# itshawi/data-accelerator

Hardware: AMD Instinct MI355X
Metric: events/sec (node) + p99 latency, SimulatedData IoT Flow (higher is better)
Workload: dtype fp64/int64 columns (no reduced precision)

## Files before the change

### dxa/ops/csrc/inflate.hip

```cpp
#include "dxa_common.h"

namespace {

constexpr int IG = 16;
constexpr int WG = 128;
constexpr int LBITS = 9;
constexpr int DBITS = 8;
constexpr int kWaitVm0 = 0xF70;

enum : int32_t { IF_OK = 0, IF_TRUNC = 1, IF_DIST = 2, IF_OVERFLOW = 3, IF_SIZE = 4, IF_CODE = 10, IF_BLOCK = 6 };

struct Tables {
  uint16_t lfast[1 << LBITS];
  uint16_t dfast[1 << DBITS];
  uint16_t lsorted[288];
  uint16_t dsorted[32];
  uint16_t lcount[16];
  uint16_t dcount[16];
  uint8_t lens[320];
  uint8_t clens[20];
  uint16_t csorted[19];
  uint16_t ccount[16];
};

__constant__ uint16_t kLenBase[29] = {3,  4,  5,  6,  7,  8,  9,  10, 11,  13,  15,  17,  19,  23, 27,
                                      31, 35, 43, 51, 59, 67, 83, 99, 115, 131, 163, 195, 227, 258};
__constant__ uint8_t kLenExtra[29] = {0, 0, 0, 0, 0, 0, 0, 0, 1, 1, 1, 1, 2, 2, 2, 2, 3, 3, 3, 3, 4, 4, 4, 4, 5, 5, 5, 5, 0};
__constant__ uint16_t kDistBase[30] = {1,   2,   3,   4,   5,   7,    9,    13,   17,   25,   33,   49,    65,    97,    129,
                                       193, 257, 385, 513, 769, 1025, 1537, 2049, 3073, 4097, 6145, 8193, 12289, 16385, 24577};
__constant__ uint8_t kDistExtra[30] = {0, 0, 0, 0, 1, 1, 2, 2, 3, 3, 4, 4, 5, 5, 6, 6, 7, 7, 8, 8, 9, 9, 10, 10, 11, 11, 12, 12, 13, 13};
__constant__ uint8_t kClenOrder[19] = {16, 17, 18, 0, 8, 7, 9, 6, 10, 5, 11, 4, 12, 3, 13, 2, 14, 1, 15};

__device__ __forceinline__ uint32_t bitrev(uint32_t c, int n) { return __builtin_bitreverse32(c) >> (32 - n); }

__device__ __forceinline__ void lane_sync() {
  __builtin_amdgcn_fence(__ATOMIC_RELEASE, "wavefront");
  __builtin_amdgcn_wave_barrier();
  __builtin_amdgcn_fence(__ATOMIC_ACQUIRE, "wavefront");
}

__device__ bool build_table(const uint8_t* lens, int n, uint16_t* count, uint16_t* sorted, uint16_t* fast, int bits,
                            int maxlen, int gl) {
  lane_sync();
  if (fast) {
    for (int i = gl; i < (1 << bits); i += IG) fast[i] = 0;
    lane_sync();
  }
  uint16_t cnt[16];
  for (int l = 0; l < 16; ++l) cnt[l] = 0;
  for (int s = 0; s < n; ++s) cnt[lens[s]]++;
  int left = 1;
  for (int l = 1; l <= maxlen; ++l) {
    left = (left << 1) - cnt[l];
    if (left < 0) return false;
  }
  uint16_t offs[16];
  offs[1] = 0;
  for (int l = 1; l < 15; ++l) offs[l + 1] = offs[l] + cnt[l];
  if (gl == 0) {
    for (int l = 0; l < 16; ++l) count[l] = cnt[l];
  }
  uint32_t next[16];
  uint32_t code = 0;
  next[0] = 0;
  for (int l = 1; l < 16; ++l) {
    next[l] = code;
    code = (code + cnt[l]) << 1;
  }
  for (int s = 0; s < n; ++s) {
    const int l = lens[s];
    if (!l) continue;
    if (gl == 0) sorted[offs[l]] = (uint16_t)s;
    offs[l]++;
    const uint32_t c = next[l]++;
    if (fast && l <= bits) {
      const uint32_t r = bitrev(c, l);
      const uint16_t e = (uint16_t)((l << 9) | s);
      for (int k = gl; k < (1 << (bits - l)); k += IG) fast[r | ((uint32_t)k << l)] = e;
    }
  }
  lane_sync();
  return true;
}

__global__ __launch_bounds__(WG) void inflate_group_kernel(const uint8_t* __restrict__ src,
                                                           const int64_t* __restrict__ comp_off,
                                                           const int32_t* __restrict__ comp_len,
                                                           const uint8_t* __restrict__ kind,
                                                           const int64_t* __restrict__ out_off,
                                                           const int64_t* __restrict__ cap_arr, int64_t nb,
                                                           uint8_t* __restrict__ dst, int64_t* __restrict__ produced,
                                                           int32_t* __restrict__ status) {
  __shared__ Tables tabs[WG / IG];
  Tables& T = tabs[threadIdx.x / IG];
  const int64_t b = ((int64_t)blockIdx.x * WG + threadIdx.x) / IG;
  const int gl = (int)(threadIdx.x & (IG - 1));
  if (b >= nb || kind[b] != 2) return;
  const uint8_t* in = src + comp_off[b];
  const int32_t n = comp_len[b];
  const int64_t cap64 = cap_arr[b];
  uint8_t* out = dst + out_off[b];
  if (n < 0 || cap64 < 0 || cap64 > INT32_MAX) {
    if (gl == 0) status[b] = IF_OVERFLOW;
    return;
  }
  const int32_t cap = (int32_t)cap64;
  const int32_t lim = n + 8;
  uint64_t bb = 0;
  int bc = 0;
  int32_t ip = 0;
  auto ld32 = [&](int32_t p) -> uint32_t {
    if (p + 4 <= lim) {
      const uintptr_t a = reinterpret_cast<uintptr_t>(in + p);
      const uint32_t* w = reinterpret_cast<const uint32_t*>(a & ~(uintptr_t)3);
      const uint32_t sh = (uint32_t)(a & 3) * 8u;
      const uint32_t lo = w[0];
      if (!sh) return lo;
      return (lo >> sh) | (w[1] << (32u - sh));
    }
    uint32_t v = 0;
    for (int i = 0; i < 4; ++i)
      if (p + i < lim) v |= (uint32_t)in[p + i] << (8 * i);
    return v;
  };
  auto refill = [&]() {
    if (bc <= 32) {
      bb |= (uint64_t)ld32(ip) << bc;
      ip += 4;
      bc += 32;
    }
  };
  auto bits = [&](int k) -> uint32_t {
    refill();
    const uint32_t v = (uint32_t)(bb & ((1ull << k) - 1));
    bb >>= k;
    bc -= k;
    return v;
  };
  auto slow = [&](const uint16_t* count, const uint16_t* sorted, int maxlen) -> int {
    refill();
    int code = 0, first = 0, index = 0;
    for (int l = 1; l <= maxlen; ++l) {
      code |= (int)(bb & 1);
      bb >>= 1;
      bc--;
      const int c = count[l];
      if (code - first < c) return sorted[index + code - first];
      index += c;
      first = (first + c) << 1;
      code <<= 1;
    }
    return -1;
  };
  auto decode = [&](const uint16_t* fast, int fbits, const uint16_t* count, const uint16_t* sorted) -> int {
    refill();
    const uint32_t e = fast[bb & ((1u << fbits) - 1)];
    const int l = (int)(e >> 9);
    if (l) {
      bb >>= l;
      bc -= l;
      return (int)(e & 511);
    }
    return slow(count, sorted, 15);
  };
  int32_t op = 0, rc = IF_OK, done = 0;
  bool last = false;
  while (!last && rc == IF_OK) {
    if ((int64_t)ip * 8 - bc > (int64_t)lim * 8) { rc = IF_TRUNC; break; }
    last = bits(1) != 0;
    const uint32_t type = bits(2);
    if (type == 0) {
      const int drop = bc & 7;
      bb >>= drop;
      bc -= drop;
      const uint32_t len = bits(16), nlen = bits(16);
      if ((len ^ 0xffffu) != nlen) { rc = IF_BLOCK; break; }
      const int32_t pos = ip - bc / 8;
      if (pos + (int32_t)len > n) { rc = IF_TRUNC; break; }
      if (op + (int32_t)len > cap) { rc = IF_OVERFLOW; break; }
      for (int32_t c = gl; c < (int32_t)len; c += IG) out[op + c] = in[pos + c];
      op += (int32_t)len;
      ip = pos + (int32_t)len;
      bb = 0;
      bc = 0;
      continue;
    }
    if (type == 3) { rc = IF_BLOCK; break; }
    int nlit = 288, ndist = 30;
    if (type == 1) {
      for (int s = gl; s < 320; s += IG) T.lens[s] = s < 144 ? 8 : s < 256 ? 9 : s < 280 ? 7 : s < 288 ? 8 : 5;
    } else {
      nlit = (int)bits(5) + 257;
      ndist = (int)bits(5) + 1;
      const int ncl = (int)bits(4) + 4;
      if (nlit > 286 || ndist > 30) { rc = IF_BLOCK; break; }
      uint32_t cl[19];
      for (int i = 0; i < 19; ++i) cl[i] = 0;
      for (int i = 0; i < ncl; ++i) cl[kClenOrder[i]] = bits(3);
      if (gl == 0) {
        for (int i = 0; i < 19; ++i) T.clens[i] = (uint8_t)cl[i];
      }
      if (!build_table(T.clens, 19, T.ccount, T.csorted, nullptr, 0, 7, gl)) { rc = IF_CODE + 0; break; }
      int i = 0;
      while (i < nlit + ndist) {
        const int sym = slow(T.ccount, T.csorted, 7);
        if (sym < 0) { rc = IF_CODE + 1; break; }
        if (sym < 16) {
          if (gl == 0) T.lens[i] = (uint8_t)sym;
          ++i;
          continue;
        }
        int rep, val = 0;
        if (sym == 16) {
          if (i == 0) { rc = IF_CODE + 2; break; }
          lane_sync();
          val = T.lens[i - 1];
          rep = 3 + (int)bits(2);
        } else if (sym == 17) {
          rep = 3 + (int)bits(3);
        } else {
          rep = 11 + (int)bits(7);
        }
        if (i + rep > nlit + ndist) { rc = IF_CODE + 3; break; }
        for (int k = gl; k < rep; k += IG) T.lens[i + k] = (uint8_t)val;
        i += rep;
      }
      if (rc != IF_OK) break;
      lane_sync();
      if (T.lens[256] == 0) { rc = IF_CODE + 4; break; }
    }
    if (!build_table(T.lens, nlit, T.lcount, T.lsorted, T.lfast, LBITS, 15, gl) ||
        !build_table(T.lens + nlit, ndist, T.dcount, T.dsorted, T.dfast, DBITS, 15, gl)) {
      rc = IF_CODE + 5;
      break;
    }
    for (;;) {
      if ((int64_t)ip * 8 - bc > (int64_t)lim * 8) { rc = IF_TRUNC; break; }
      const int sym = decode(T.lfast, LBITS, T.lcount, T.lsorted);
      if (sym < 0) { rc = IF_CODE + 6; break; }
      if (sym < 256) {
        if (op >= cap) { rc = IF_OVERFLOW; break; }
        if (gl == 0) out[op] = (uint8_t)sym;
        ++op;
        continue;
      }
      if (sym == 256) break;
      const int li = sym - 257;
      if (li >= 29) { rc = IF_CODE + 7; break; }
      const int32_t len = kLenBase[li] + (int32_t)bits(kLenExtra[li]);
      const int ds = decode(T.dfast, DBITS, T.dcount, T.dsorted);
      if (ds < 0 || ds >= 30) { rc = IF_CODE + 8; break; }
      const int32_t dist = kDistBase[ds] + (int32_t)bits(kDistExtra[ds]);
      if (dist > op) { rc = IF_DIST; break; }
      if (len > cap - op) { rc = IF_OVERFLOW; break; }
      const int32_t s0 = op - dist;
      if (s0 + (dist < len ? dist : len) > done) {
        __builtin_amdgcn_s_waitcnt(kWaitVm0);
        asm volatile("" ::: "memory");
        done = op;
      }
      if (dist >= len) {
        for (int32_t c = 0; c < len; c += IG)
          if (c + gl < len) out[op + c + gl] = out[s0 + c + gl];
      } else {
        for (int32_t c = 0; c < len; c += IG) {
          const uint32_t k = (uint32_t)(c + gl);
          if ((int32_t)k < len) out[op + (int32_t)k] = out[s0 + (int32_t)(k % (uint32_t)dist)];
        }
      }
      op += len;
    }
  }
  if (rc == IF_OK && op != cap) rc = IF_SIZE;
  if (gl == 0) {
    status[b] = rc;
    produced[b] = op;
  }
}

}

DXA_API int dxa_inflate_into(const void* src, const void* comp_off, const void* comp_len, const void* kind,
                             const void* out_off, const void* cap, int64_t nb, void* dst, void* produced, void* status,
                             void* st) {
  if (nb <= 0) return 0;
  hipLaunchKernelGGL(inflate_group_kernel, dim3((unsigned)((nb * IG + WG - 1) / WG)), dim3(WG), 0, (hipStream_t)st,
                     (const uint8_t*)src, (const int64_t*)comp_off, (const int32_t*)comp_len, (const uint8_t*)kind,
                     (const int64_t*)out_off, (const int64_t*)cap, nb, (uint8_t*)dst, (int64_t*)produced,
                     (int32_t*)status);
  return (int)hipGetLastError();
}
```

Measured before the change: 252.1 million.

## Rework inflate bit reader, table build and literal stores in GPU decoder

Replaces the per-refill unaligned 32-bit loads with a 16-byte windowed prefetch reader, and swaps bit-by-bit slow Huffman decoding for a canonical limit-table search. Table building now counts code lengths cooperatively with LDS atomics and shares one count array, and the code-length table reuses the literal fast table. Length and distance bases are computed arithmetically instead of read from constant memory. Literals are buffered across lanes and written as one group store instead of a single-lane byte store each. It also pins waves-per-EU occupancy. The cost is added register pressure and more complex edge handling for the window near buffer bounds.

```diff
diff --git a/dxa/ops/csrc/inflate.hip b/dxa/ops/csrc/inflate.hip
--- a/dxa/ops/csrc/inflate.hip
+++ b/dxa/ops/csrc/inflate.hip
@@ -1,12 +1,24 @@
 #include "dxa_common.h"
 
+#ifndef DXA_INFLATE_IG
+#define DXA_INFLATE_IG 16
+#endif
+#ifndef DXA_INFLATE_WG
+#define DXA_INFLATE_WG 128
+#endif
+#ifndef DXA_INFLATE_LBITS
+#define DXA_INFLATE_LBITS 9
+#endif
+
 namespace {
 
-constexpr int IG = 16;
-constexpr int WG = 128;
-constexpr int LBITS = 9;
+constexpr int IG = DXA_INFLATE_IG;
+constexpr int WG = DXA_INFLATE_WG;
+constexpr int LBITS = DXA_INFLATE_LBITS;
 constexpr int DBITS = 8;
+constexpr int CBITS = 7;
 constexpr int kWaitVm0 = 0xF70;
+static_assert(LBITS >= CBITS && LBITS <= 11 && (IG == 8 || IG == 16 || IG == 32), "table / group shape");
 
 enum : int32_t { IF_OK = 0, IF_TRUNC = 1, IF_DIST = 2, IF_OVERFLOW = 3, IF_SIZE = 4, IF_CODE = 10, IF_BLOCK = 6 };
 
@@ -15,23 +27,35 @@
   uint16_t dfast[1 << DBITS];
   uint16_t lsorted[288];
   uint16_t dsorted[32];
-  uint16_t lcount[16];
-  uint16_t dcount[16];
+  uint32_t count[16];
   uint8_t lens[320];
-  uint8_t clens[20];
-  uint16_t csorted[19];
-  uint16_t ccount[16];
 };
 
-__constant__ uint16_t kLenBase[29] = {3,  4,  5,  6,  7,  8,  9,  10, 11,  13,  15,  17,  19,  23, 27,
-                                      31, 35, 43, 51, 59, 67, 83, 99, 115, 131, 163, 195, 227, 258};
-__constant__ uint8_t kLenExtra[29] = {0, 0, 0, 0, 0, 0, 0, 0, 1, 1, 1, 1, 2, 2, 2, 2, 3, 3, 3, 3, 4, 4, 4, 4, 5, 5, 5, 5, 0};
-__constant__ uint16_t kDistBase[30] = {1,   2,   3,   4,   5,   7,    9,    13,   17,   25,   33,   49,    65,    97,    129,
-                                       193, 257, 385, 513, 769, 1025, 1537, 2049, 3073, 4097, 6145, 8193, 12289, 16385, 24577};
-__constant__ uint8_t kDistExtra[30] = {0, 0, 0, 0, 1, 1, 2, 2, 3, 3, 4, 4, 5, 5, 6, 6, 7, 7, 8, 8, 9, 9, 10, 10, 11, 11, 12, 12, 13, 13};
 __constant__ uint8_t kClenOrder[19] = {16, 17, 18, 0, 8, 7, 9, 6, 10, 5, 11, 4, 12, 3, 13, 2, 14, 1, 15};
 
+typedef uint32_t u32x4 __attribute__((ext_vector_type(4), aligned(4)));
+
 __device__ __forceinline__ uint32_t bitrev(uint32_t c, int n) { return __builtin_bitreverse32(c) >> (32 - n); }
+
+__device__ __forceinline__ uint32_t window_dword(const uint4& w, uint32_t k) {
+  const uint64_t lo = ((uint64_t)w.y << 32) | w.x;
+  const uint64_t hi = ((uint64_t)w.w << 32) | w.z;
+  const uint64_t x = (k & 2u) ? hi : lo;
+  return (uint32_t)(x >> ((k & 1u) * 32u));
+}
+
+__device__ __forceinline__ uint4 load_window_edge(const uint8_t* __restrict__ a0, int32_t q, int32_t lo, int32_t lim) {
+  uint64_t h[2] = {0, 0};
+#pragma unroll
+  for (int k = 0; k < 2; ++k) {
+#pragma unroll 1
+    for (int i = 0; i < 8; ++i) {
+      const int32_t p = q + 8 * k + i;
+      if (p >= lo && p < lim) h[k] |= (uint64_t)a0[p] << (8 * i);
+    }
+  }
+  return make_uint4((uint32_t)h[0], (uint32_t)(h[0] >> 32), (uint32_t)h[1], (uint32_t)(h[1] >> 32));
+}
 
 __device__ __forceinline__ void lane_sync() {
   __builtin_amdgcn_fence(__ATOMIC_RELEASE, "wavefront");
@@ -39,58 +63,82 @@
   __builtin_amdgcn_fence(__ATOMIC_ACQUIRE, "wavefront");
 }
 
-__device__ bool build_table(const uint8_t* lens, int n, uint16_t* count, uint16_t* sorted, uint16_t* fast, int bits,
-                            int maxlen, int gl) {
+template <int FB>
+__device__ __forceinline__ bool build_table(const uint8_t* lens, int n, uint32_t* count, uint16_t* sorted,
+                                            uint16_t* fast, int gl, uint32_t (&lim)[16 - FB]) {
   lane_sync();
-  if (fast) {
-    for (int i = gl; i < (1 << bits); i += IG) fast[i] = 0;
-    lane_sync();
-  }
-  uint16_t cnt[16];
-  for (int l = 0; l < 16; ++l) cnt[l] = 0;
-  for (int s = 0; s < n; ++s) cnt[lens[s]]++;
+#pragma unroll 1
+  for (int i = gl; i < (1 << FB); i += IG) fast[i] = 0;
+  for (int l = gl; l < 16; l += IG) count[l] = 0;
+  lane_sync();
+#pragma unroll 1
+  for (int s = gl; s < n; s += IG)
+    __hip_atomic_fetch_add(&count[lens[s]], 1u, __ATOMIC_RELAXED, __HIP_MEMORY_SCOPE_WORKGROUP);
+  lane_sync();
+  uint32_t cnt[16];
+#pragma unroll
+  for (int l = 0; l < 16; ++l) cnt[l] = count[l];
   int left = 1;
-  for (int l = 1; l <= maxlen; ++l) {
+  for (int l = 1; l <= 15; ++l) {
     left = (left << 1) - cnt[l];
     if (left < 0) return false;
   }
-  uint16_t offs[16];
-  offs[1] = 0;
-  for (int l = 1; l < 15; ++l) offs[l + 1] = offs[l] + cnt[l];
-  if (gl == 0) {
-    for (int l = 0; l < 16; ++l) count[l] = cnt[l];
-  }
   uint32_t next[16];
-  uint32_t code = 0;
+  uint32_t code = 0, off = 0;
   next[0] = 0;
+#pragma unroll
   for (int l = 1; l < 16; ++l) {
-    next[l] = code;
-    code = (code + cnt[l]) << 1;
-  }
+    next[l] = code | (off << 16);
+    code += cnt[l];
+    off += cnt[l];
+    if (l >= FB) lim[l - FB] = (code << (15 - l)) | (off << 16);
+    code <<= 1;
+  }
+#pragma unroll 1
   for (int s = 0; s < n; ++s) {
     const int l = lens[s];
     if (!l) continue;
-    if (gl == 0) sorted[offs[l]] = (uint16_t)s;
-    offs[l]++;
-    const uint32_t c = next[l]++;
-    if (fast && l <= bits) {
-      const uint32_t r = bitrev(c, l);
+    const uint32_t c = next[l];
+    next[l] = c + 0x10001u;
+    if (gl == 0) sorted[c >> 16] = (uint16_t)s;
+    if (l <= FB) {
+      const uint32_t r = bitrev(c & 0xffffu, l);
       const uint16_t e = (uint16_t)((l << 9) | s);
-      for (int k = gl; k < (1 << (bits - l)); k += IG) fast[r | ((uint32_t)k << l)] = e;
+      for (int k = gl; k < (1 << (FB - l)); k += IG) fast[r | ((uint32_t)k << l)] = e;
     }
   }
   lane_sync();
   return true;
 }
 
-__global__ __launch_bounds__(WG) void inflate_group_kernel(const uint8_t* __restrict__ src,
-                                                           const int64_t* __restrict__ comp_off,
-                                                           const int32_t* __restrict__ comp_len,
-                                                           const uint8_t* __restrict__ kind,
-                                                           const int64_t* __restrict__ out_off,
-                                                           const int64_t* __restrict__ cap_arr, int64_t nb,
-                                                           uint8_t* __restrict__ dst, int64_t* __restrict__ produced,
-                                                           int32_t* __restrict__ status) {
+template <int FB>
+__device__ __forceinline__ int decode_sym(uint64_t& bb, int& bc, const uint16_t* fast, const uint16_t* sorted,
+                                          const uint32_t (&lim)[16 - FB]) {
+  const uint32_t e = fast[(uint32_t)bb & ((1u << FB) - 1)];
+  int l = (int)(e >> 9);
+  int sym = (int)(e & 511);
+  if (!l) {
+    const uint32_t c = __builtin_bitreverse32((uint32_t)bb) >> 17;
+    if (c >= (lim[15 - FB] & 0xffffu)) return -1;
+    l = FB + 1;
+    uint32_t base = lim[0];
+#pragma unroll
+    for (int j = 1; j < 15 - FB; ++j) {
+      const bool longer = c >= (lim[j] & 0xffffu);
+      l += longer ? 1 : 0;
+      base = longer ? lim[j] : base;
+    }
+    sym = sorted[(base >> 16) + ((c - (base & 0xffffu)) >> (15 - l))];
+  }
+  bb >>= l;
+  bc -= l;
+  return sym;
+}
+
+__global__ __launch_bounds__(WG) __attribute__((amdgpu_waves_per_eu(4, 4))) void inflate_group_kernel(
+    const uint8_t* __restrict__ src, const int64_t* __restrict__ comp_off, const int32_t* __restrict__ comp_len,
+    const uint8_t* __restrict__ kind, const int64_t* __restrict__ out_off, const int64_t* __restrict__ cap_arr,
+    int64_t nb, uint8_t* __restrict__ dst, int64_t* __restrict__ produced, int32_t* __restrict__ status) {
   __shared__ Tables tabs[WG / IG];
   Tables& T = tabs[threadIdx.x / IG];
   const int64_t b = ((int64_t)blockIdx.x * WG + threadIdx.x) / IG;
@@ -100,35 +148,52 @@
   const int32_t n = comp_len[b];
   const int64_t cap64 = cap_arr[b];
   uint8_t* out = dst + out_off[b];
-  if (n < 0 || cap64 < 0 || cap64 > INT32_MAX) {
+  if (n < 0 || n > INT32_MAX - 64 || cap64 < 0 || cap64 > INT32_MAX) {
     if (gl == 0) status[b] = IF_OVERFLOW;
     return;
   }
   const int32_t cap = (int32_t)cap64;
-  const int32_t lim = n + 8;
+  const int32_t lo = (int32_t)(reinterpret_cast<uintptr_t>(in) & 3);
+  const uint8_t* a0 = in - lo;
+  const int32_t lim = lo + n + 8;
+  auto whole = [&](int32_t q) { return q >= lo && q + 16 <= lim; };
   uint64_t bb = 0;
   int bc = 0;
   int32_t ip = 0;
-  auto ld32 = [&](int32_t p) -> uint32_t {
-    if (p + 4 <= lim) {
-      const uintptr_t a = reinterpret_cast<uintptr_t>(in + p);
-      const uint32_t* w = reinterpret_cast<const uint32_t*>(a & ~(uintptr_t)3);
-      const uint32_t sh = (uint32_t)(a & 3) * 8u;
-      const uint32_t lo = w[0];
-      if (!sh) return lo;
-      return (lo >> sh) | (w[1] << (32u - sh));
-    }
-    uint32_t v = 0;
-    for (int i = 0; i < 4; ++i)
-      if (p + i < lim) v |= (uint32_t)in[p + i] << (8 * i);
-    return v;
+  uint4 cur;
+  u32x4 nxt = {0, 0, 0, 0};
+  int32_t wb = 0;
+  auto open_window = [&]() {
+    if (whole(wb)) cur = make_uint4(nxt.x, nxt.y, nxt.z, nxt.w);
+    else cur = load_window_edge(a0, wb, lo, lim);
+    if (whole(wb + 16)) nxt = *reinterpret_cast<const u32x4*>(a0 + wb + 16);
+  };
+  auto seek = [&](int32_t p) {
+    wb = p & ~15;
+    if (whole(wb)) nxt = *reinterpret_cast<const u32x4*>(a0 + wb);
+    open_window();
+    ip = p & ~3;
+    const int sh = (p & 3) * 8;
+    bb = window_dword(cur, (uint32_t)(ip - wb) >> 2) >> sh;
+    bc = 32 - sh;
+    ip += 4;
   };
   auto refill = [&]() {
     if (bc <= 32) {
-      bb |= (uint64_t)ld32(ip) << bc;
+      if (ip - wb == 16) {
+        wb += 16;
+        open_window();
+      }
+      bb |= (uint64_t)window_dword(cur, (uint32_t)(ip - wb) >> 2) << bc;
       ip += 4;
       bc += 32;
     }
+  };
+  auto take = [&](int k) -> uint32_t {
+    const uint32_t v = (uint32_t)(bb & ((1ull << k) - 1));
+    bb >>= k;
+    bc -= k;
+    return v;
   };
   auto bits = [&](int k) -> uint32_t {
     refill();
@@ -137,36 +202,19 @@
     bc -= k;
     return v;
   };
-  auto slow = [&](const uint16_t* count, const uint16_t* sorted, int maxlen) -> int {
-    refill();
-    int code = 0, first = 0, index = 0;
-    for (int l = 1; l <= maxlen; ++l) {
-      code |= (int)(bb & 1);
-      bb >>= 1;
-      bc--;
-      const int c = count[l];
-      if (code - first < c) return sorted[index + code - first];
-      index += c;
-      first = (first + c) << 1;
-      code <<= 1;
-    }
-    return -1;
-  };
-  auto decode = [&](const uint16_t* fast, int fbits, const uint16_t* count, const uint16_t* sorted) -> int {
-    refill();
-    const uint32_t e = fast[bb & ((1u << fbits) - 1)];
-    const int l = (int)(e >> 9);
-    if (l) {
-      bb >>= l;
-      bc -= l;
-      return (int)(e & 511);
-    }
-    return slow(count, sorted, 15);
-  };
+  auto past_end = [&]() { return ip > lim && (ip - lim) * 8 > bc; };
   int32_t op = 0, rc = IF_OK, done = 0;
+  uint32_t mine = 0;
+  int nacc = 0;
+  auto flush = [&]() {
+    if (gl < nacc) out[op - nacc + gl] = (uint8_t)mine;
+    nacc = 0;
+  };
+  uint32_t llim[16 - LBITS], dlim[16 - DBITS];
+  seek(lo);
   bool last = false;
   while (!last && rc == IF_OK) {
-    if ((int64_t)ip * 8 - bc > (int64_t)lim * 8) { rc = IF_TRUNC; break; }
+    if (past_end()) { rc = IF_TRUNC; break; }
     last = bits(1) != 0;
     const uint32_t type = bits(2);
     if (type == 0) {
@@ -176,13 +224,12 @@
       const uint32_t len = bits(16), nlen = bits(16);
       if ((len ^ 0xffffu) != nlen) { rc = IF_BLOCK; break; }
       const int32_t pos = ip - bc / 8;
-      if (pos + (int32_t)len > n) { rc = IF_TRUNC; break; }
+      if (pos - lo + (int32_t)len > n) { rc = IF_TRUNC; break; }
       if (op + (int32_t)len > cap) { rc = IF_OVERFLOW; break; }
-      for (int32_t c = gl; c < (int32_t)len; c += IG) out[op + c] = in[pos + c];
+      flush();
+      for (int32_t c = gl; c < (int32_t)len; c += IG) out[op + c] = a0[pos + c];
       op += (int32_t)len;
-      ip = pos + (int32_t)len;
-      bb = 0;
-      bc = 0;
+      seek(pos + (int32_t)len);
       continue;
     }
     if (type == 3) { rc = IF_BLOCK; break; }
@@ -194,16 +241,21 @@
       ndist = (int)bits(5) + 1;
       const int ncl = (int)bits(4) + 4;
       if (nlit > 286 || ndist > 30) { rc = IF_BLOCK; break; }
-      uint32_t cl[19];
-      for (int i = 0; i < 19; ++i) cl[i] = 0;
-      for (int i = 0; i < ncl; ++i) cl[kClenOrder[i]] = bits(3);
-      if (gl == 0) {
-        for (int i = 0; i < 19; ++i) T.clens[i] = (uint8_t)cl[i];
-      }
-      if (!build_table(T.clens, 19, T.ccount, T.csorted, nullptr, 0, 7, gl)) { rc = IF_CODE + 0; break; }
+      lane_sync();
+      for (int i = gl; i < 19; i += IG) T.lens[i] = 0;
+      lane_sync();
+#pragma unroll 1
+      for (int i = 0; i < ncl; ++i) {
+        const uint32_t v = bits(3);
+        if (gl == 0) T.lens[kClenOrder[i]] = (uint8_t)v;
+      }
+      uint32_t clim[16 - CBITS];
+      if (!build_table<CBITS>(T.lens, 19, T.count, T.lsorted, T.lfast, gl, clim)) { rc = IF_CODE + 0; break; }
       int i = 0;
+#pragma unroll 1
       while (i < nlit + ndist) {
-        const int sym = slow(T.ccount, T.csorted, 7);
+        refill();
+        const int sym = decode_sym<CBITS>(bb, bc, T.lfast, T.lsorted, clim);
         if (sym < 0) { rc = IF_CODE + 1; break; }
         if (sym < 16) {
           if (gl == 0) T.lens[i] = (uint8_t)sym;
@@ -229,30 +281,38 @@
       lane_sync();
       if (T.lens[256] == 0) { rc = IF_CODE + 4; break; }
     }
-    if (!build_table(T.lens, nlit, T.lcount, T.lsorted, T.lfast, LBITS, 15, gl) ||
-        !build_table(T.lens + nlit, ndist, T.dcount, T.dsorted, T.dfast, DBITS, 15, gl)) {
+    if (!build_table<LBITS>(T.lens, nlit, T.count, T.lsorted, T.lfast, gl, llim) ||
+        !build_table<DBITS>(T.lens + nlit, ndist, T.count, T.dsorted, T.dfast, gl, dlim)) {
       rc = IF_CODE + 5;
       break;
     }
     for (;;) {
-      if ((int64_t)ip * 8 - bc > (int64_t)lim * 8) { rc = IF_TRUNC; break; }
-      const int sym = decode(T.lfast, LBITS, T.lcount, T.lsorted);
+      if (past_end()) { rc = IF_TRUNC; break; }
+      refill();
+      const int sym = decode_sym<LBITS>(bb, bc, T.lfast, T.lsorted, llim);
       if (sym < 0) { rc = IF_CODE + 6; break; }
       if (sym < 256) {
         if (op >= cap) { rc = IF_OVERFLOW; break; }
-        if (gl == 0) out[op] = (uint8_t)sym;
+        if (gl == nacc) mine = (uint32_t)sym;
         ++op;
+        if (++nacc == IG) flush();
         continue;
       }
       if (sym == 256) break;
       const int li = sym - 257;
       if (li >= 29) { rc = IF_CODE + 7; break; }
-      const int32_t len = kLenBase[li] + (int32_t)bits(kLenExtra[li]);
-      const int ds = decode(T.dfast, DBITS, T.dcount, T.dsorted);
+      const int le = (li < 8 || li == 28) ? 0 : (li - 4) >> 2;
+      const int32_t lbase = li < 8 ? 3 + li : li == 28 ? 258 : 3 + ((4 + (li & 3)) << le);
+      const int32_t len = lbase + (int32_t)take(le);
+      refill();
+      const int ds = decode_sym<DBITS>(bb, bc, T.dfast, T.dsorted, dlim);
       if (ds < 0 || ds >= 30) { rc = IF_CODE + 8; break; }
-      const int32_t dist = kDistBase[ds] + (int32_t)bits(kDistExtra[ds]);
+      const int de = ds < 4 ? 0 : (ds - 2) >> 1;
+      const int32_t dbase = ds < 4 ? 1 + ds : 1 + ((2 + (ds & 1)) << de);
+      const int32_t dist = dbase + (int32_t)take(de);
       if (dist > op) { rc = IF_DIST; break; }
       if (len > cap - op) { rc = IF_OVERFLOW; break; }
+      flush();
       const int32_t s0 = op - dist;
       if (s0 + (dist < len ? dist : len) > done) {
         __builtin_amdgcn_s_waitcnt(kWaitVm0);
@@ -271,6 +331,7 @@
       op += len;
     }
   }
+  flush();
   if (rc == IF_OK && op != cap) rc = IF_SIZE;
   if (gl == 0) {
     status[b] = rc;
```

Result: no change. 251.9 million (median of 2 runs) (-0.1%).
